# AdaptiveCity/deepdish

Measured on AMD Instinct MI355X. Metric: end-to-end frames/sec (detect+encode+track) at 640x480, higher is better.
Workload: dtype i8 (reference: uint8); encoder f16; 1 GPU; SSD-MobileNet-v1 uint8-quantised (300x300) + MARS-64x32x3 + deep_sort on synthetic 640x480 BGR frames, ~20 synthetic detections/frame (BASELINE.json configs[1]); streams_per_gpu=3072, worker_threads_per_gpu=2, parallelism=independent streams, 3072 per GPU in 2 worker groups, weights=seeded synthetic (seed 1234)

## Files before the change

deepdish_amd/csrc/mars_pair.hip:

```cpp
#include "mars_tail.h"

namespace {

typedef _Float16 h8 __attribute__((ext_vector_type(8)));
typedef float f4 __attribute__((ext_vector_type(4)));
typedef unsigned u4 __attribute__((ext_vector_type(4)));

__device__ __forceinline__ float elu(float v) {
    float e = __builtin_amdgcn_exp2f(v * 1.44269504088896340736f);
    e = __builtin_amdgcn_fmed3f(e, 0.f, 1.f);
    return __builtin_amdgcn_fmed3f(v, e - 1.f, 3.0e38f);
}

__device__ __forceinline__ void lds_fill16(const _Float16 *g, char *lds_wave_base) {
#if defined(__HIP_DEVICE_COMPILE__)
    __builtin_amdgcn_global_load_lds(g, lds_wave_base, 16, 0, 0);
#endif
}

__device__ __forceinline__ int frag_row(int a, int fr) { return (fr >> 2) * 8 + (a & 1) * 4 + (fr & 3); }

constexpr int PZ_B = 3072;
constexpr int PT64_B = 18 * 1024;
constexpr int PT32_B = 33 * 1024;
// ... 43 lines not shown
                    const size_t row = (size_t)(half * 32 + frag_row(a, fr)) * kpad;
                    wf[t][ks][a] = a32 ? *reinterpret_cast<const h8 *>(w + row + t * 32 + fq * 8)
                                       : *reinterpret_cast<const h8 *>(w + row + t * 64 + ks * 32 + fq * 8);
                }
#pragma unroll
        for (int a = 0; a < 2; ++a)
            wp[a] = FIRST ? *reinterpret_cast<const h8 *>(P.wp + (size_t)(half * 32 + frag_row(a, fr)) * P.kpad_p + fq * 8) : wf[0][0][a];
    }
#if defined(__HIP_DEVICE_COMPILE__)
#pragma unroll
    for (int t = 0; t < 9; ++t)
#pragma unroll
        for (int ks = 0; ks < 2; ++ks)
#pragma unroll
            for (int a = 0; a < 2; ++a) asm volatile("" ::"v"(wf[t][ks][a]));
    asm volatile("" ::"v"(wp[0]), "v"(wp[1]));
#endif

    const int n0 = blockIdx.x, nstep = gridDim.x;
    const int Kc = (P.n_img - n0 + nstep - 1) / nstep;

    const _Float16 *src[5];
    size_t stp[5];
    int n_dma;
    if constexpr (FIRST) {
        const int par = lane >> 5, pl = (lane >> 3) & 3, col = 2 * (lane & 7) + par;
#pragma unroll
        for (int h = 0; h < 4; ++h) {
            const int r = wave + 8 * h < 31 ? wave + 8 * h : 30;
            src[h] = col < 15 ? P.in + ((size_t)n0 * 31 + r) * 15 * P.cs_in + (size_t)col * P.cs_in + P.coff_in + pl * 8 : P.zero;
            stp[h] = col < 15 ? (size_t)nstep * 31 * 15 * P.cs_in : 0;
        }
        const int jr = lane >> 5, xx = lane & 7;
        src[4] = P.in2 + ((size_t)n0 * 31 + 2 * (2 * wave + jr)) * 15 * P.cs_in2 + (size_t)(2 * xx) * P.cs_in2 + P.coff_in2 + pl * 8;
        stp[4] = (size_t)nstep * 31 * 15 * P.cs_in2;
        n_dma = 5;
    } else {
        const int pl = lane >> 3, xx = lane & 7;
#pragma unroll
        for (int h = 0; h < 2; ++h) {
            src[h] = P.in + (((size_t)n0 * 16 + wave + 8 * h) * 8 + xx) * P.cs_in + P.coff_in + pl * 8;
            stp[h] = (size_t)nstep * 128 * P.cs_in;
            src[2 + h] = P.res + (((size_t)n0 * 16 + wave + 8 * h) * 8 + xx) * P.cs_res + P.coff_res + pl * 8;
            stp[2 + h] = (size_t)nstep * 128 * P.cs_res;
        }
        src[4] = P.zero; stp[4] = 0;
        n_dma = 4;
    }
    (void)n_dma;
    int dq = 0;
    auto issue = [&]() {
        char *T = smem + OFF_IN + (dq & 1) * TIN_B;
        if constexpr (FIRST) {
#pragma unroll
            for (int h = 0; h < 4; ++h) lds_fill16(src[h], T + ((wave + 8 * h < 31 ? wave + 8 * h : 30) + 1) * 1024);
            lds_fill16(src[4], smem + OFF_RAW + (dq & 1) * PRAW_B + wave * 1024);
        } else {
#pragma unroll
            for (int h = 0; h < 2; ++h) lds_fill16(src[h], T + (wave + 8 * h + 1) * 1024);
            const int rs = dq % 3;
#pragma unroll
            for (int h = 0; h < 2; ++h) lds_fill16(src[2 + h], smem + OFF_RES + rs * PPLAIN_B + (wave + 8 * h) * 1024);
        }
        ++dq;
        const bool more = dq < Kc;
#pragma unroll
        for (int h = 0; h < 5; ++h) src[h] += more ? stp[h] : 0;
    };
// ... 46 lines not shown
            } else {
                const unsigned tb = (unsigned)((stage == 0 ? OFF_IN + (cc & 1) * PT64_B : OFF_H + (cc & 1) * PT64_B) + 2 * F * 1024) + lo64;
                const unsigned bL = x == 0 ? ((tb - 16u) & 255u) : tb - 16u, bC = tb, bR = x == 7 ? ((tb + 16u) & 255u) : tb + 16u;
#if defined(__HIP_DEVICE_COMPILE__)
#define DD_RD(u_) do { constexpr int t_ = (u_) >> 1, ks_ = (u_) & 1, dy_ = t_ / 3, dx_ = t_ - dy_ * 3;                                             \
                       asm volatile("ds_read_b128 %0, %1 offset:%2" : "=&v"(X[(u_) & 3]) : "v"(dx_ == 0 ? bL : dx_ == 1 ? bC : bR), "n"(dy_ * 1024 + ks_ * 512) : "memory"); } while (0)
#define DD_UNIT(u_) do { if constexpr ((u_) + 3 < 18) DD_RD(((u_) + 3) % 18);                                                                      \
                         asm volatile("s_waitcnt lgkmcnt(%1)" : "+v"(X[(u_) & 3]) : "n"((u_) + 3 < 18 ? 3 : 17 - (u_)));                          \
                         _Pragma("unroll") for (int a = 0; a < 2; ++a) acc[a] = __builtin_amdgcn_mfma_f32_16x16x32_f16(wf[(u_) >> 1][(u_) & 1][a], X[(u_) & 3], acc[a], 0, 0, 0); } while (0)
                DD_RD(0); DD_RD(1); DD_RD(2);
                DD_UNIT(0); DD_UNIT(1); DD_UNIT(2); DD_UNIT(3); DD_UNIT(4); DD_UNIT(5); DD_UNIT(6); DD_UNIT(7); DD_UNIT(8);
                DD_UNIT(9); DD_UNIT(10); DD_UNIT(11); DD_UNIT(12); DD_UNIT(13); DD_UNIT(14); DD_UNIT(15); DD_UNIT(16); DD_UNIT(17);
#undef DD_UNIT
#undef DD_RD
#endif
            }
            float v[8];
#pragma unroll
            for (int i = 0; i < 4; ++i) { v[i] = acc[0][i] + ba0[i]; v[4 + i] = acc[1][i] + ba1[i]; }
            if (stage == 0) {
                h8 o;
#pragma unroll
                for (int i = 0; i < 8; ++i) o[i] = (_Float16)elu(v[i]);
                *reinterpret_cast<h8 *>(smem + OFF_H + (cc & 1) * PT64_B + ((2 * F + j + 1) * 64 + (half * 4 + fq) * 8 + x) * 16) = o;
            } else {
                const int rs = FIRST ? (cc & 1) : cc % 3;
                const h8 rv = *reinterpret_cast<const h8 *>(smem + OFF_RES + rs * PPLAIN_B + ((2 * F + j) * 64 + (half * 4 + fq) * 8 + x) * 16);
#pragma unroll
                for (int i = 0; i < 8; ++i) v[i] += (float)rv[i];
                const size_t m = (n * 16 + 2 * F + j) * 8 + x;
                h8 o;
#pragma unroll
                for (int i = 0; i < 8; ++i) o[i] = (_Float16)v[i];
                *reinterpret_cast<h8 *>(P.out + m * P.cs_out + P.coff_out + co) = o;
                const f4 s0 = *reinterpret_cast<const f4 *>(cst + 128 + co), s1 = *reinterpret_cast<const f4 *>(cst + 128 + co + 4);
                const f4 t0 = *reinterpret_cast<const f4 *>(cst + 192 + co), t1 = *reinterpret_cast<const f4 *>(cst + 192 + co + 4);
                h8 o2;
#pragma unroll
                for (int i = 0; i < 4; ++i) { o2[i] = (_Float16)elu(s0[i] * v[i] + t0[i]); o2[4 + i] = (_Float16)elu(s1[i] * v[4 + i] + t1[i]); }
                *reinterpret_cast<h8 *>(P.out2 + m * P.cs_out2 + P.coff_out2 + co) = o2;
            }
        }
    }
#if defined(__HIP_DEVICE_COMPILE__)
    asm volatile("s_waitcnt vmcnt(0)" ::: "memory");
#endif
}

template <bool FIRST>
int launch_pair(hipStream_t s, int device, const MarsPairP &P) {
    constexpr int lds = pair_lds_bytes(FIRST);
    static_assert(lds <= 160 * 1024, "LDS budget");
    static DevOnce once;
    const int rc = once.run(device, [&]() -> int {
        DD_HIP(hipFuncSetAttribute(reinterpret_cast<const void *>(&mars_pair64_k<FIRST>), hipFuncAttributeMaxDynamicSharedMemorySize, lds));
        return DD_OK;
    });
    if (rc != DD_OK) return rc;
    const int n_cu = dd_cu_count(device);
    const int grid = P.n_img < n_cu ? P.n_img : n_cu;
    hipLaunchKernelGGL((mars_pair64_k<FIRST>), dim3(grid), dim3(512), lds, s, P);
    DD_LAUNCH_CHECK();
    return DD_OK;
}

}

// ... 6 lines not shown
```

deepdish_amd/csrc/mars_tail.h:

```cpp
#pragma once
#include "common.h"

struct MarsWsP {
    const _Float16 *in;  int cs_in, coff_in;
    const _Float16 *in2; int cs_in2, coff_in2;
    const _Float16 *w;   int kpad;
    const _Float16 *w2;  int kpad2;
    const float *bias, *bias2;
    const _Float16 *res; int cs_res, coff_res;
    _Float16 *out;  int cs_out, coff_out;
    _Float16 *out2; int cs_out2, coff_out2;
    const float *aff2; int cout_pad;
    const _Float16 *zero;
    int n_img;
};

enum { MARS_WS_S1 = 0, MARS_WS_S1_RES = 1, MARS_WS_S2_PROJ = 2 };

int mars_ws128_launch(hipStream_t s, int device, const MarsWsP &P, int mode, int act, bool out2);

struct MarsPairP {
    const _Float16 *in;  int cs_in, coff_in;
    const _Float16 *in2; int cs_in2, coff_in2;
    const _Float16 *wa;  int kpad_a; const float *bias_a;
    const _Float16 *wp;  int kpad_p; const float *bias_p;
    const _Float16 *wb;  int kpad_b; const float *bias_b;
    const _Float16 *res; int cs_res, coff_res;
    _Float16 *out;  int cs_out, coff_out;
    _Float16 *out2; int cs_out2, coff_out2;
    const float *aff2; int cout_pad;
    const _Float16 *zero;
    int n_img;
};
int mars_pair64_launch(hipStream_t s, int device, const MarsPairP &P, bool first);
```

deepdish_amd/csrc/mars_tail.hip:

```cpp
#include "mars_tail.h"
#include <vector>

namespace {

typedef _Float16 h8 __attribute__((ext_vector_type(8)));
typedef float f4 __attribute__((ext_vector_type(4)));
typedef unsigned u4 __attribute__((ext_vector_type(4)));

enum { ACT_NONE = 0, ACT_ELU = 2 };

__device__ __forceinline__ float elu(float v) {
    float e = __builtin_amdgcn_exp2f(v * 1.44269504088896340736f);
    e = __builtin_amdgcn_fmed3f(e, 0.f, 1.f);
    return __builtin_amdgcn_fmed3f(v, e - 1.f, 3.0e38f);
}

__device__ __forceinline__ void lds_fill16(const _Float16 *g, char *lds_wave_base) {
#if defined(__HIP_DEVICE_COMPILE__)
    __builtin_amdgcn_global_load_lds(g, lds_wave_base, 16, 0, 0);
#endif
}

__device__ __forceinline__ int frag_row(int a, int fr) { return (fr >> 2) * 8 + (a & 1) * 4 + (fr & 3); }

// ... 51 lines not shown
                wf[t][ks][a] = *reinterpret_cast<const h8 *>(P.w + (size_t)(cg * 32 + frag_row(a, fr)) * P.kpad + t * CIN + kh * (CIN / 2) + ks * 32 + fq * 8);
    h8 wp[2];
    if constexpr (S2) {
#pragma unroll
        for (int a = 0; a < 2; ++a) wp[a] = *reinterpret_cast<const h8 *>(P.w2 + (size_t)(cg * 32 + frag_row(a, fr)) * P.kpad2 + kh * 32 + fq * 8);
    }

#if defined(__HIP_DEVICE_COMPILE__)
#pragma unroll
    for (int t = 0; t < 9; ++t)
#pragma unroll
        for (int ks = 0; ks < KS; ++ks)
#pragma unroll
            for (int a = 0; a < 2; ++a) asm volatile("" ::"v"(wf[t][ks][a]));
    if constexpr (S2) asm volatile("" ::"v"(wp[0]), "v"(wp[1]));
#endif

    const int n0 = blockIdx.x, nstep = gridDim.x;
    const int Kc = (P.n_img - n0 + nstep - 1) / nstep;

    int dq = 0, dq_slot = 0, dq_rslot = 0;
    const _Float16 *src_a, *src_b, *src_c;
    size_t step_a, step_b, step_c;
    if constexpr (!S2) {
        src_a = P.in + (size_t)n0 * 32 * P.cs_in + ((wave * 4 + (lane & 3)) * P.cs_in + P.coff_in + (lane >> 2) * 8);
        src_b = RES ? P.res + (size_t)n0 * 32 * P.cs_res + ((wave * 4 + (lane & 3)) * P.cs_res + P.coff_res + (lane >> 2) * 8) : P.zero;
        src_c = P.zero;
        step_a = (size_t)nstep * 32 * P.cs_in; step_b = (size_t)nstep * 32 * P.cs_res; step_c = 0;
    } else {
        const int par = lane >> 5, pl = (lane >> 2) & 7, col = 2 * (lane & 3) + par;
        src_a = P.in + (size_t)n0 * 128 * P.cs_in + ((wave * 8 + col) * P.cs_in + P.coff_in + pl * 8);
        src_b = src_a + (size_t)64 * P.cs_in;
        const int ch = (wave & 3) * 64 + lane;
        src_c = P.in2 + (size_t)n0 * 128 * P.cs_in2 + ((2 * ((ch >> 2) & 7) * 8 + 2 * (ch & 3)) * P.cs_in2 + P.coff_in2 + (ch >> 5) * 8);
        step_a = step_b = (size_t)nstep * 128 * P.cs_in; step_c = (size_t)nstep * 128 * P.cs_in2;
    }
    auto issue = [&]() {
        char *T = smem + OFF_T + dq_slot * TILE_B;
        if constexpr (!S2) {
            lds_fill16(src_a, T + (wave + 1) * 72 * 16);
            if constexpr (RES) lds_fill16(src_b, smem + OFF_A + dq_rslot * WS_RES_BYTES + wave * 72 * 16);
        } else {
            lds_fill16(src_a, T + wave * 68 * 16);
            lds_fill16(src_b, T + (wave + 8) * 68 * 16);
            lds_fill16(src_c, smem + OFF_A + dq_slot * WS_PRJ_BYTES + (wave & 3) * 1024);
        }
        ++dq;
        const bool more = dq < Kc;
        src_a += more ? step_a : 0;
        if constexpr (RES || S2) src_b += more ? step_b : 0;
        if constexpr (S2) src_c += more ? step_c : 0;
        dq_slot = dq_slot + 1 == NB ? 0 : dq_slot + 1;
        dq_rslot = dq_rslot + 1 == NBR ? 0 : dq_rslot + 1;
    };

    const unsigned lo = S2 ? (unsigned)((2 * yy * 68 + (kh * 4 + fq) * 4 + x) * 16) : (unsigned)((yy * 72 + (kh * 8 + fq) * 4 + x) * 16);
    const unsigned lo_prj = (unsigned)(((kh * 4 + fq) * 32 + yy * 4 + x) * 16);
    const unsigned lo_res = (unsigned)(((4 * kh + yy) * 72 + (cg * 4 + fq) * 4 + x) * 16);
    const int co = cg * 32 + fq * 8;
    const f4 b0 = *reinterpret_cast<const f4 *>(cst + co), b1 = *reinterpret_cast<const f4 *>(cst + co + 4);

    f4 keep[S2 ? 4 : 2];
    int slot = 0, rslot_prev = 0, rslot = 0;

    auto epilogue = [&](int cprev) {
        const char *Xp = smem + OFF_X + ((cprev & 1) * 8 + (wave ^ 4)) * XW_B + lane * 16;
        const size_t n = (size_t)(n0 + cprev * nstep);
        const size_t m = (n * 8 + 4 * kh + yy) * 4 + x;
// ... 209 lines not shown
```

deepdish_amd/csrc/net_priv.h:

```cpp
#pragma once
#include <map>
#include <utility>
#include <vector>
#include "common.h"

struct TensorDesc { int buf, h, w, c, cs, coff, dtype, pad; };

struct dd_net {
    dd_ctx *ctx = nullptr;
    int max_batch = 0;
    std::vector<int32_t> prog;
    std::vector<TensorDesc> tensors;
    std::vector<int64_t> buf_elems;
    std::vector<void *> bufs;
    std::vector<int> buf_dtype;
    int n_ops = 0, ops_off = 0;
    void *arena = nullptr;
    int64_t arena_bytes = 0;
    char *d_weights = nullptr;
    int64_t weight_bytes = 0;
    int in_h = 0, in_w = 0, out_tensor = -1;
    bool profile = false;
    int last_batch = 0;
    DevBuf slab;
    bool ssd_dec = false, yolo_dec = false;
    int dec_anchors = 0; float dec_thr = 0.f;
    float *d_anchors = nullptr, *dec_boxes = nullptr, *dec_score = nullptr, *dec_keys = nullptr; int *dec_cls = nullptr;
    bool slab_moved = false;
    _Float16 *d_zero = nullptr;
    std::vector<hipEvent_t> events;
    std::vector<int32_t> op_launch;
    std::vector<int32_t> op_variant;
    struct GraphEntry { int calls = 0; hipGraph_t graph = nullptr; hipGraphExec_t exec = nullptr; };
    bool use_graph = false;
    std::map<std::pair<const void *, int>, GraphEntry> graphs;
};

constexpr int OP_WORDS = 48;
constexpr int TENSOR_WORDS = 8;

enum { OP_INPUT = 1, OP_CONV = 2, OP_DWCONV = 3, OP_MAXPOOL = 4, OP_UPSAMPLE = 5, OP_FC = 6, OP_L2NORM = 7, OP_STEM = 8, OP_DWPW = 9 };
enum { OP_QCONV0 = 16, OP_QCONV = 17, OP_QDW = 18, OP_QDWPW = 19, OP_QSSD_DECODE = 20, OP_QADD = 21 };
enum { ACT_NONE = 0, ACT_RELU6 = 1, ACT_ELU = 2, ACT_SILU = 3, ACT_RELU = 4, ACT_SIGMOID = 5 };
enum { EPI_F16 = 0, EPI_F32 = 1, EPI_SSD_HEAD = 2, EPI_YOLO = 3 };
enum { DT_F16 = 0, DT_F32 = 1, DT_U8 = 2 };
enum { HINT_NONE = 0,
       HINT_NEXT_ONLY = 1,
       HINT_HOLD_UNIT = 2,
       HINT_NEXT_IS_PROJ = 3,
       HINT_PAIR_MEMBER = 4 };

enum OpWord {
    W_KIND = 0,
    W_SRC = 1,
    W_DST = 2,
    W_RES = 3,
    W_DST2 = 4,
    W_KH = 5,
    W_KW = 6,
    W_STRIDE = 7,
    W_PAD_T = 8,
    W_PAD_L = 9,
    W_CIN = 10,
    W_COUT = 11,
    W_COUT_PAD = 12,
// ... 123 lines not shown
```

deepdish_amd/csrc/nets.hip:

```cpp
#include <algorithm>
#include <cmath>
#include <cstdlib>
#include <map>
#include <string>
#include "common.h"
#include "ssd_dev.h"
#include "net_priv.h"
#include "mars_tail.h"

namespace {

typedef _Float16 h8 __attribute__((ext_vector_type(8)));
typedef _Float16 h4 __attribute__((ext_vector_type(4)));
typedef float f4 __attribute__((ext_vector_type(4)));

enum { OPK_DEFAULT = 0, OPK_FOLDED = 1, OPK_POOL_ROWS = 2, OPK_POOL_ROWS_STEM = 3, OPK_RES_UNIT = 4, OPK_SSD_FRONT = 5, OPK_C64_ROWS = 6, OPK_S2_ROWS = 7, OPK_CONV_WS = 8, OPK_WS_DW = 9, OPK_DWPW_ROWS = 10, OPK_SSD_HEAD_DEC = 11, OPK_RES_PAIR = 12, OPK_YOLO_HEAD_DEC = 13, OPK_MARS_WS = 14, OPK_FOLDED_PREV = 15, OPK_MARS_PAIR = 16, OPK_C64_STRIPS = 18, OPK_Q_FRONT = 19, OPK_Q_MID = 20, OPK_STEM_WIDE = 23 };

__device__ __forceinline__ float fast_sigmoid(float v) { return __builtin_amdgcn_rcpf(1.f + __expf(-v)); }

__device__ __forceinline__ float yolo_box_col(int o, float s, float px, float py, float stride, float aw, float ah, float img_w, float img_h) {
#pragma clang fp contract(off)
    if (o == 0) return (s * 2.f - 0.5f + px) * stride / img_w;
    if (o == 1) return (s * 2.f - 0.5f + py) * stride / img_h;
    if (o == 2) return (s * 2.f) * (s * 2.f) * aw / img_w;
// ... 6 lines not shown
        case ACT_ELU: {
            float e = __builtin_amdgcn_exp2f(v * 1.44269504088896340736f);
            e = __builtin_amdgcn_fmed3f(e, 0.f, 1.f);
            return __builtin_amdgcn_fmed3f(v, e - 1.f, 3.0e38f);
        }
        case ACT_SILU: {
            float r = v * fast_sigmoid(v);
#if defined(__HIP_DEVICE_COMPILE__)
            asm("" : "+v"(r));
#endif
            return r;
        }
        case ACT_RELU: return fmaxf(v, 0.f);
        case ACT_SIGMOID: return 1.f / (1.f + __expf(-v));
        default: return v;
    }
}

__device__ __forceinline__ float pool_max(float a, float b) {
#if defined(__HIP_DEVICE_COMPILE__)
    return __builtin_elementwise_maximum(a, b);
#else
    return a > b ? a : b;
#endif
}

struct ConvP {
    const _Float16 *in; int H, W, cs_in, coff_in, cin;
    const _Float16 *w; const float *bias; int kpad;
    int kh, kw, stride, pad_t, pad_l;
    int ho, wo, cout, m;
    int act;
    void *out; int cs_out, coff_out, epi;
    const _Float16 *res; int cs_res, coff_res;
    _Float16 *out2; int cs_out2, coff_out2; const float *aff2; int cout_pad;
    int post_aff;
    int splitk; float *slab;
    const _Float16 *zero;
    int p[6]; float f[8];
    int th, tw, tiles_x, tiles_y;
    const uint8_t *src8; float in_mean, in_scale;
    const _Float16 *dw_w; const float *dw_bias; int dw_act; int total_quads;
    const float *anchors; float *dec_boxes, *dec_score, *dec_keys; int *dec_cls; float dec_thr;
};


__device__ __forceinline__ void conv_epilogue(const ConvP &P, int m, int co, float v[4], int hw) {
    const f4 bv = *reinterpret_cast<const f4 *>(P.bias + co);
#pragma unroll
    for (int r = 0; r < 4; ++r) v[r] += bv[r];
    if (P.epi == EPI_YOLO) {
        const int n = m / hw, p = m - n * hw;
        const int py = p / P.wo, px = p - py * P.wo;
#pragma unroll
        for (int r = 0; r < 4; ++r) {
            const int ch = co + r;
            if (ch >= P.cout) continue;
            const int no = P.p[0];
            const int an = ch / no, o = ch - an * no;
            const float s = fast_sigmoid(v[r]);
            float val = s;
            if (o < 4) val = yolo_box_col(o, s, (float)px, (float)py, P.f[6], P.f[2 * an], P.f[2 * an + 1], P.f[7], (float)P.p[4]);
            const size_t row = (size_t)n * P.p[1] + P.p[2] + (size_t)an * hw + p;
            static_cast<float *>(P.out)[row * no + o] = val;
        }
        return;
// ... 55 lines not shown
#if defined(__HIP_DEVICE_COMPILE__)
    if (HI) asm("v_fma_mix_f32 %0, %1, %2, %0 op_sel:[1,1,0] op_sel_hi:[1,1,0]" : "+v"(acc) : "v"(x), "v"(w));
    else asm("v_fma_mix_f32 %0, %1, %2, %0 op_sel:[0,0,0] op_sel_hi:[1,1,0]" : "+v"(acc) : "v"(x), "v"(w));
#endif
    return acc;
}
__device__ __forceinline__ void dw_tap(float (&acc)[8], const h8 &x, const h8 &w) {
    const u4v_t xv = __builtin_bit_cast(u4v_t, x), wv = __builtin_bit_cast(u4v_t, w);
#pragma unroll
    for (int i = 0; i < 8; ++i)
        acc[i] = (i & 1) ? fma_mix_f16<1>(xv[i >> 1], wv[i >> 1], acc[i]) : fma_mix_f16<0>(xv[i >> 1], wv[i >> 1], acc[i]);
}

struct Epi8 { f4 b0, b1, s0, s1, t0, t1; };

__device__ __forceinline__ Epi8 epi8_load(const ConvP &P, int co) {
    Epi8 E;
    E.b0 = *reinterpret_cast<const f4 *>(P.bias + co);
    E.b1 = *reinterpret_cast<const f4 *>(P.bias + co + 4);
    E.s0 = E.s1 = E.t0 = E.t1 = f4{0.f, 0.f, 0.f, 0.f};
    if (P.out2) {
        E.s0 = *reinterpret_cast<const f4 *>(P.aff2 + co);
        E.s1 = *reinterpret_cast<const f4 *>(P.aff2 + co + 4);
        E.t0 = *reinterpret_cast<const f4 *>(P.aff2 + P.cout_pad + co);
        E.t1 = *reinterpret_cast<const f4 *>(P.aff2 + P.cout_pad + co + 4);
    }
    return E;
}

#ifndef DD_EPI_NT
#define DD_EPI_NT true
#endif
template <int ACT = -1, bool BIAS = true, int EF = -1, bool NT = DD_EPI_NT, bool TAIL = true>
__device__ __forceinline__ void conv_epilogue_f16x8(const ConvP &P, const Epi8 &E, int m, int co, float v[8], const h8 *res_pre = nullptr) {
    const int act = ACT < 0 ? P.act : ACT;
    const bool has_res = EF < 0 ? P.res != nullptr : EF >= 1, has_out2 = EF < 0 ? P.out2 != nullptr : EF == 1;
#pragma unroll
    for (int r = 0; r < 4; ++r) {
        v[r] = apply_act(BIAS ? v[r] + E.b0[r] : v[r], act);
        v[4 + r] = apply_act(BIAS ? v[4 + r] + E.b1[r] : v[4 + r], act);
    }
    if (has_res) {
        const h8 rv = res_pre ? *res_pre : *reinterpret_cast<const h8 *>(P.res + (size_t)m * P.cs_res + P.coff_res + co);
#pragma unroll
        for (int r = 0; r < 8; ++r) v[r] += (float)rv[r];
    }
    const bool tail = TAIL && co + 8 > P.cout;
    h8 o;
#pragma unroll
    for (int r = 0; r < 8; ++r) o[r] = (_Float16)v[r];
    if (tail) {
#pragma unroll
        for (int r = 0; r < 8; ++r)
            if (co + r >= P.cout) o[r] = (_Float16)0.f;
    }
    h8 *dst = reinterpret_cast<h8 *>(static_cast<_Float16 *>(P.out) + (size_t)m * P.cs_out + P.coff_out + co);
    if constexpr (NT) __builtin_nontemporal_store(o, dst);
    else *dst = o;
    if (has_out2) {
        h8 o2;
#pragma unroll
        for (int r = 0; r < 8; ++r) {
            const float sc = r < 4 ? E.s0[r] : E.s1[r - 4], sh = r < 4 ? E.t0[r] : E.t1[r - 4];
            o2[r] = (_Float16)apply_act(sc * v[r] + sh, ACT_ELU);
        }
        if (tail) {
#pragma unroll
            for (int r = 0; r < 8; ++r)
                if (co + r >= P.cout) o2[r] = (_Float16)0.f;
        }
        *reinterpret_cast<h8 *>(P.out2 + (size_t)m * P.cs_out2 + P.coff_out2 + co) = o2;
    }
}

template <int ACT = -1>
__device__ __forceinline__ void conv_epilogue_f16x8(const ConvP &P, int m, int co, float v[8]) {
    const Epi8 E = epi8_load(P, co);
    conv_epilogue_f16x8<ACT>(P, E, m, co, v);
}

template <int ACT, int BM, int BN, int T>
__device__ __forceinline__ void conv_finish_rows(const ConvP &P, const float *ot, int m0, int n0) {
    constexpr int OROW = BN + 4, G = BN / 8;
    static_assert(T % G == 0, "a thread keeps its channel group over the row loop");
    const int g = threadIdx.x % G, co = n0 + g * 8;
    if (co >= P.cout_pad) return;
    const Epi8 E = epi8_load(P, co);
    for (int pl = threadIdx.x / G; pl < BM; pl += T / G) {
        const int m = m0 + pl;
        if (m >= P.m) break;
        const f4 lo = *reinterpret_cast<const f4 *>(ot + pl * OROW + g * 8);
// ... 1387 lines not shown
            __builtin_amdgcn_sched_barrier(0);
#endif
            if (i + 1 < 4) rd(i + 1, X[(i + 1) & 1]);
#if defined(__HIP_DEVICE_COMPILE__)
            __builtin_amdgcn_sched_barrier(0);
#endif
#pragma unroll
            for (int dx = 0; dx < 3; ++dx)
#pragma unroll
                for (int cr = 0; cr < 2; ++cr) {
                    const int dy = i - cr;
                    if (dy < 0 || dy > 2) continue;
#pragma unroll
                    for (int a = 0; a < 2; ++a)
                        acc[cr][a] = __builtin_amdgcn_mfma_f32_16x16x32_f16(w[dy * 3 + dx][a], x[dx], acc[cr][a], 0, 0, 0);
                }
#if defined(__HIP_DEVICE_COMPILE__)
            __builtin_amdgcn_sched_barrier(0);
#endif
        }
    };
    f4 accC[2][2];
    int grC = -1;
    auto b_store = [&]() {
#pragma unroll
        for (int cr = 0; cr < 2; ++cr) {
            const int s = 2 * grC - 1 + cr;
            const int kk = (s + 1) >> 5, y = ((s + 1) & 31) - 1;
            if (y < 0 || fr >= W) continue;
            float o[8];
#pragma unroll
            for (int q = 0; q < 4; ++q) { o[q] = accC[cr][0][q]; o[4 + q] = accC[cr][1][q]; }
            const h8 rv = *reinterpret_cast<const h8 *>(resr + ((s + 1) & (RU_PRE_SLOTS - 1)) * RU_SLOT + offC);
            conv_epilogue_f16x8<ACT_NONE, false, 1, true, false>(P2B, EB, ((n0 + kk * nstep) * H + y) * W + fr, fq * 8, o, &rv);
        }
    };
    for (int g = 0; g < Gall; ++g) {
        const int gr = role ? g - 2 : g;
        const bool active = role ? (gr >= 0 && gr < GA) : (K > 0 && gr <= GA);
        if (grC >= 0) { b_store(); grC = -1; }
        if (active) {
            if (role == 0) { fill_pre(2 * gr + 5); fill_pre(2 * gr + 6); }
            {
                f4 acc[2][2] = {{bA0, bA1}, {bA0, bA1}};
                conv2(inr, 2 * gr, RU_PRE_SLOTS - 1, wA, acc);
#pragma unroll
                for (int cr = 0; cr < 2; ++cr) {
                    const int s = 2 * gr + cr;
                    const bool live = ((s + 1) & 31) != 0 && fr < W;
                    h8 o;
#pragma unroll
                    for (int q = 0; q < 4; ++q) {
                        o[q] = (_Float16)apply_act(acc[cr][0][q], actA);
                        o[4 + q] = (_Float16)apply_act(acc[cr][1][q], actA);
                    }
                    u4v_t ou = __builtin_bit_cast(u4v_t, o);
                    ou &= live ? 0xFFFFFFFFu : 0u;
                    *reinterpret_cast<u4v_t *>(h1r + (s & (RU_H1_SLOTS - 1)) * RU_SLOT + offC) = ou;
                }
            }
            {
                f4 acc[2][2] = {{EB.b0, EB.b1}, {EB.b0, EB.b1}};
                conv2(h1r, 2 * gr - 2, RU_H1_SLOTS - 1, wB, acc);
                h8 rv[2];
#pragma unroll
                for (int cr = 0; cr < 2; ++cr) rv[cr] = *reinterpret_cast<const h8 *>(resr + ((2 * gr + cr) & (RU_PRE_SLOTS - 1)) * RU_SLOT + offC);
                if (role == 0) {
// ... 2337 lines not shown
    *n_ops_host = n->n_ops;
    return DD_OK;
}

int dd_net_op_variants(dd_net *n, int32_t *codes_host, int cap, int *n_ops_host) {
    DD_REQUIRE(n && codes_host && n_ops_host, DD_E_ARG, "dd_net_op_variants: NULL argument");
    DD_REQUIRE(cap >= n->n_ops, DD_E_ARG, "dd_net_op_variants: cap %d < %d ops", cap, n->n_ops);
    for (int i = 0; i < n->n_ops; ++i) codes_host[i] = i < (int)n->op_variant.size() ? n->op_variant[i] : 0;
    *n_ops_host = n->n_ops;
    return DD_OK;
}

int dd_net_read(dd_net *n, int tensor, int n_img, void *dst, int dst_on_device, void *stream) {
    DD_REQUIRE(n && dst && n_img >= 0 && n_img <= n->max_batch, DD_E_ARG, "dd_net_read: bad argument");
    DD_DEVICE(n->ctx);
    const int t = tensor < 0 ? n->out_tensor : tensor;
    DD_REQUIRE(t >= 0 && t < (int)n->tensors.size(), DD_E_ARG, "dd_net_read: tensor %d out of range", t);
    const TensorDesc &d = n->tensors[t];
    DD_REQUIRE(!n->arena || t == n->out_tensor, DD_E_STATE, "dd_net_read: tensor %d of an engine whose buffers share memory by lifetime "
               "(dd_net_create_shared): only the output tensor outlives the forward", t);
    DD_REQUIRE(d.coff == 0, DD_E_ARG, "dd_net_read: tensor %d is a channel slice", t);
    for (int i = 0; i < n->n_ops && i < (int)n->op_launch.size(); ++i) {
        const OpView o = op(n, i);
        DD_REQUIRE(!(o.dst() == t && n->op_launch[i] == OPK_SSD_HEAD_DEC), DD_E_STATE,
                   "dd_net_read: tensor %d (the SSD head matrix) was not written: the head layers decoded in their epilogue "
                   "(dd_net_ssd_decode); read dd_net_ssd_decoded instead", t);
        DD_REQUIRE(!(o.dst() == t && n->op_launch[i] == OPK_YOLO_HEAD_DEC), DD_E_STATE,
                   "dd_net_read: tensor %d (the Detect matrix) was not written: the head layers reduced their rows in their epilogue "
                   "(dd_net_yolo_decode); read dd_net_yolo_decoded instead", t);
        DD_REQUIRE(!((o.dst() == t || o.dst2() == t) && n->op_launch[i] == OPK_FOLDED), DD_E_STATE,
                   "dd_net_read: tensor %d was not written by the last forward (op %d ran inside the next op's launch at this batch "
                   "size and its output stayed on chip); run a smaller batch or a program compiled without the fusion flags", t, i);
    }
    hipStream_t s = dd_pick_stream(n->ctx, stream);
    const size_t bytes = d.pad ? (size_t)n_img * (d.h + 2) * (d.w + 2) * d.cs
                               : (size_t)n_img * d.h * d.w * d.cs * dtype_size(d.dtype);
    if (!bytes) return DD_OK;
    DD_HIP(hipMemcpyAsync(dst, n->bufs[d.buf], bytes, dst_on_device ? hipMemcpyDeviceToDevice : hipMemcpyDeviceToHost, s));
    if (!dst_on_device) DD_HIP(hipStreamSynchronize(s));
    return DD_OK;
}

static int net_run_ops(dd_net *net, const uint8_t *input, int nimg, hipStream_t s);

int dd_net_use_graph(dd_net *net, int enable) {
    DD_REQUIRE(net, DD_E_ARG, "dd_net_use_graph: NULL net");
    DD_DEVICE(net->ctx);
    net->use_graph = enable != 0;
    if (!net->use_graph) net_drop_graphs(net);
    return DD_OK;
}

int dd_net_ssd_decode(dd_net *net, const float *anchors_host, int n_anchors, float score_thr, int enable) {
    DD_REQUIRE(net, DD_E_ARG, "dd_net_ssd_decode: NULL net");
    DD_DEVICE(net->ctx);
    net_drop_graphs(net);
    if (!enable) { net->ssd_dec = false; return DD_OK; }
    DD_REQUIRE(anchors_host && n_anchors > 0, DD_E_ARG, "dd_net_ssd_decode: anchors missing");
    int heads = 0;
    for (int i = 0; i < net->n_ops; ++i) {
        const OpView o = op(net, i);
        if (o.kind() == OP_CONV && o.epi() == EPI_SSD_HEAD) {
            DD_REQUIRE(o.aff_off() && o.p(1) == n_anchors && 4 + o.p(0) <= 96, DD_E_ARG,
                       "dd_net_ssd_decode: head op %d has no per-anchor weight copy, or %d anchors / %d classes do not fit", i, o.p(1), o.p(0));
            ++heads;
        }
// ... 198 lines not shown
    DD_REQUIRE(!h.unit_on && !h.pair_on && !h.stem_on && !h.pw_on && !h.input_on, DD_E_STATE,
               "dd_net_forward: op %d is folded into a neighbouring launch while an earlier op's launch is still held back", i);
    return DD_OK;
}

ConvP conv_params(const dd_net *net, const OpView &o, int nimg) {
    ConvP P;
    memset(&P, 0, sizeof(P));
    if (o.src() >= 0) {
        bind_tensor(net, o.src(), P.in, P.cs_in, P.coff_in);
        P.H = net->tensors[o.src()].h; P.W = net->tensors[o.src()].w;
    }
    P.cin = o.cin();
    P.kh = o.kh(); P.kw = o.kw(); P.stride = o.stride(); P.pad_t = o.pad_t(); P.pad_l = o.pad_l();
    P.cout = o.cout(); P.cout_pad = o.cout_pad(); P.kpad = o.kpad(); P.act = o.act(); P.epi = o.epi();
    P.w = blob<_Float16>(net, o.w_off());
    P.bias = blob<float>(net, o.bias_off());
    P.ho = o.ho(); P.wo = o.wo(); P.m = nimg * P.ho * P.wo;
    bind_tensor(net, o.dst(), P.out, P.cs_out, P.coff_out);
    if (o.res() >= 0) bind_tensor(net, o.res(), P.res, P.cs_res, P.coff_res);
    if (o.dst2() >= 0) {
        bind_tensor(net, o.dst2(), P.out2, P.cs_out2, P.coff_out2);
        P.aff2 = blob<float>(net, o.aff_off());
    }
    if (o.dst2() < 0 && o.has_aff()) {
        P.aff2 = blob<float>(net, o.aff_off());
        P.post_aff = 1;
    }
    for (int q = 0; q < 6; ++q) P.p[q] = o.p(q);
    for (int q = 0; q < 8; ++q) P.f[q] = o.f(q);
    return P;
}

void take_stem(ConvP &P, const ConvP &stem) {
    P.src8 = stem.src8; P.in_mean = stem.in_mean; P.in_scale = stem.in_scale;
    P.dw_w = stem.w; P.dw_bias = stem.bias; P.dw_act = stem.act;
}

bool unit_first_layer(const Run &r, int i, const OpView &o, const ConvP &P) {
    return o.hint() != HINT_NONE && !o.pool() && i + 1 < r.net->n_ops && r.nimg >= 160 && !P.res && !P.out2;
}

int run_input(Run &r, int i, const OpView &o) {
    dd_net *net = r.net; Held &h = r.held; hipStream_t s = r.s;
    const int dst = o.dst();
    const TensorDesc *td = &net->tensors[dst];
    _Float16 *out; int cs, coff;
    bind_tensor(net, dst, out, cs, coff);
    const int m = r.nimg * td->h * td->w;
    if (o.s2d() && o.hint() != HINT_NONE && !o.swap_rb() && cs == 32 && !coff && i + 1 < net->n_ops) {
        static const bool off = dd_env_int("DD_FOCUS_UNFUSED", 0) != 0;
        if (!off && rw_shape_plain(op(net, i + 1), dst, ACT_SILU) && td->w % 32 == 0) {
            h.input_on = true; h.input_mean = o.f(0); h.input_scale = o.f(1); h.input_op = i;
            net->op_launch[i] = OPK_FOLDED;
            return DD_OK;
        }
    }
    if (o.s2d() && cs >= 16 && cs % 8 == 0) {
        const int cpp = cs / 8;
        DD_REQUIRE((long long)m * cpp < (1ll << 31), DD_E_CAPACITY, "dd_net_forward: %d x %d input chunks", m, cpp);
        hipLaunchKernelGGL(input_s2d_chunks_k, dim3(dd_ceil_div(m * cpp, 256)), dim3(256), 0, s, r.input, net->in_h, net->in_w, o.swap_rb(),
                           o.f(0), o.f(1), m * cpp, cpp, out + coff, cs);
    } else
    hipLaunchKernelGGL(input_k, dim3(dd_ceil_div(m, 256)), dim3(256), 0, s, r.input, net->in_h, net->in_w, o.swap_rb(),
                       o.f(0), o.f(1), o.s2d(), m, out + coff, cs);
    DD_LAUNCH_CHECK();
// ... 42 lines not shown
            h.stem_on = false;
            take_stem(P, h.stem);
        } else if ((rc = flush(r, HELD_STEM)) != DD_OK) return rc;
    }
    if (unit_first_layer(r, i, o, P)) {
        if (h.pair_on && P.in != static_cast<const _Float16 *>(h.pair_b.out2) && (rc = flush(r, HELD_PAIR)) != DD_OK) return rc;
        h.unit_a = P; h.unit_op = i; h.unit_on = true;
        net->op_launch[i] = OPK_FOLDED;
        return DD_OK;
    }
    if (o.pool() && pool_rows_fusable(P, nimg)) net->op_launch[i] = P.src8 ? OPK_POOL_ROWS_STEM : OPK_POOL_ROWS;
    return launch_conv3x3_rw(r.s, P, nimg, o.pool(), r.device());
}

int run_conv(Run &r, int i, const OpView &o) {
    dd_net *net = r.net; Held &h = r.held; const int nimg = r.nimg; hipStream_t s = r.s;
    int rc;
    if (h.proj_done) {
        if ((rc = refuse_fold_while_held(h, i)) != DD_OK) return rc;
        h.proj_done = false; net->op_launch[i] = OPK_FOLDED_PREV;
        return DD_OK;
    }
    if (h.pair64_left > 0) {
        if ((rc = refuse_fold_while_held(h, i)) != DD_OK) return rc;
        if (--h.pair64_left > 0) { net->op_launch[i] = OPK_FOLDED; return DD_OK; }
        if ((rc = mars_pair64_launch(s, r.device(), h.pair64, h.pair64_first)) != DD_OK) return rc;
        net->op_launch[i] = OPK_MARS_PAIR;
        return DD_OK;
    }
    if (o.hint() == HINT_NEXT_IS_PROJ || o.hint() == HINT_PAIR_MEMBER) {
        const int n_ops = mars_pair_match(net, i, nimg, h.pair64, h.pair64_first);
        if (n_ops) {
            if ((rc = refuse_fold_while_held(h, i)) != DD_OK) return rc;
            h.pair64_left = n_ops - 1; net->op_launch[i] = OPK_FOLDED;
            return DD_OK;
        }
    }
    ConvP P = conv_params(net, o, nimg);
    DD_REQUIRE(!o.pool() || (P.kh == 3 && P.stride == 1 && P.cin == 32 && P.cout_pad == 32), DD_E_ARG,
               "dd_net_forward: fused pooling is only built for the 3x3 32->32 kernel");
    if (h.unit_on) {
        if (res_unit_fusable(h.unit_a, P, nimg)) {
            h.unit_on = false;
            P.zero = net->d_zero;
            if (h.pair_on) {
                if (res_pair_fusable(h.pair_a, h.pair_b, h.unit_a, P, nimg)) {
                    h.pair_on = false;
                    if ((rc = launch_res_pair(s, h.pair_a, h.pair_b, h.unit_a, P, nimg, r.device())) != DD_OK) return rc;
                    net->op_launch[i] = OPK_RES_PAIR;
                    return DD_OK;
                }
                if ((rc = flush(r, HELD_PAIR)) != DD_OK) return rc;
            }
            if (o.hint() == HINT_HOLD_UNIT && i + 2 < net->n_ops) {
                h.pair_a = h.unit_a; h.pair_b = P; h.pair_on = true; h.pair_op = i;
                net->op_launch[i] = OPK_FOLDED;
                return DD_OK;
            }
            if ((rc = launch_res_unit(s, h.unit_a, P, nimg, r.device())) != DD_OK) return rc;
            net->op_launch[i] = OPK_RES_UNIT;
            return DD_OK;
        }
        if (h.pair_on && (rc = flush(r, HELD_PAIR)) != DD_OK) return rc;
        if ((rc = flush(r, HELD_UNIT)) != DD_OK) return rc;
    }
    if (h.pair_on) {
        const bool next_a = rw_shape(P) && unit_first_layer(r, i, o, P) && P.in == static_cast<const _Float16 *>(h.pair_b.out2);
        if (!next_a && (rc = flush(r, HELD_PAIR)) != DD_OK) return rc;
    }
    if (P.epi == EPI_YOLO && net->yolo_dec && o.aff_off() && !o.has_aff()) {
        DD_REQUIRE(P.p[1] == net->dec_anchors, DD_E_ARG, "dd_net_forward: head of %d rows, decode set up for %d", P.p[1], net->dec_anchors);
        P.w = blob<_Float16>(net, o.aff_off());
        P.bias = blob<float>(net, o.aux_off());
        P.zero = net->d_zero;
        P.dec_boxes = net->dec_boxes; P.dec_score = net->dec_score; P.dec_cls = net->dec_cls;
        if ((rc = launch_yolo_head_dec(s, P)) != DD_OK) return rc;
        net->op_launch[i] = OPK_YOLO_HEAD_DEC;
        return DD_OK;
    }
    if (P.epi == EPI_SSD_HEAD && net->ssd_dec && o.aff_off() && !o.has_aff()) {
        DD_REQUIRE(P.p[1] == net->dec_anchors, DD_E_ARG, "dd_net_forward: head of %d anchors, decode set up for %d", P.p[1], net->dec_anchors);
        P.w = blob<_Float16>(net, o.aff_off());
        P.bias = blob<float>(net, o.aux_off());
        P.zero = net->d_zero;
        P.anchors = net->d_anchors; P.dec_boxes = net->dec_boxes; P.dec_score = net->dec_score; P.dec_keys = net->dec_keys;
        P.dec_cls = net->dec_cls; P.dec_thr = net->dec_thr;
        if ((rc = launch_ssd_head_dec(s, P)) != DD_OK) return rc;
        net->op_launch[i] = OPK_SSD_HEAD_DEC;
        return DD_OK;
    }
    const bool bk32 = o.bk() == 32;
    P.zero = net->d_zero;
    if (rw_shape(P)) return run_conv3x3_rw(r, i, o, P);
    if (mars_ws_s1_eligible(P)) {
        const MarsWsP Q = mars_ws_params(P, nimg);
        net->op_launch[i] = OPK_MARS_WS;
        return mars_ws128_launch(s, r.device(), Q, P.res ? MARS_WS_S1_RES : MARS_WS_S1, P.act, P.out2 != nullptr);
    } else if (o.hint() == HINT_NEXT_IS_PROJ && i + 1 < net->n_ops && mars_ws_s2_eligible(P) && mars_proj_follows(net, i, P)) {
        const OpView q = op(net, i + 1);
        MarsWsP Q = mars_ws_params(P, nimg);
        bind_tensor(net, q.src(), Q.in2, Q.cs_in2, Q.coff_in2);
        Q.w2 = blob<_Float16>(net, q.w_off()); Q.kpad2 = q.kpad();
        Q.bias2 = blob<float>(net, q.bias_off());
        bind_tensor(net, q.dst(), Q.out2, Q.cs_out2, Q.coff_out2);
        net->op_launch[i] = OPK_MARS_WS;
        rc = mars_ws128_launch(s, r.device(), Q, MARS_WS_S2_PROJ, P.act, false);
        h.proj_done = true;
        return rc;
    } else if (s2_rows_eligible(P, nimg, net->max_batch)) {
        net->op_launch[i] = OPK_S2_ROWS;
        return launch_conv3x3_s2_rows(s, P, nimg, r.device());
    } else if (c64_rows_eligible(P, nimg, net->max_batch)) {
        net->op_launch[i] = OPK_C64_ROWS;
        return launch_conv3x3_c64_rows(s, P, nimg, r.device());
    } else if (c64_strips_eligible(P, nimg, net->max_batch)) {
        net->op_launch[i] = OPK_C64_STRIPS;
        return launch_conv3x3_c64_strips(s, P, nimg, r.device());
    } else if (ws_eligible(P) && o.hint() != HINT_NONE && i + 1 < net->n_ops && P.act == ACT_RELU6) {
        h.pw = P; h.pw_op = i; h.pw_on = true; net->op_launch[i] = OPK_FOLDED;
        return DD_OK;
    } else if (ws_eligible(P)) {
        net->op_launch[i] = OPK_CONV_WS;
        return launch_ws(r, P);
    }
    return launch_conv_tiled(r, i, P, bk32);
}

int run_stem(Run &r, int i, const OpView &o) {
    dd_net *net = r.net; Held &h = r.held; const int nimg = r.nimg;
    const int dst = o.dst();
    const TensorDesc *td = &net->tensors[dst];
    ConvP P = conv_params(net, o, nimg);
    P.src8 = r.input; P.H = net->in_h; P.W = net->in_w; P.in_mean = o.f(0); P.in_scale = o.f(1);
    P.zero = net->d_zero;
// ... 157 lines not shown
    dd_net *net = r.net; const int nimg = r.nimg; hipStream_t s = r.s;
    const bool front_on = dd_env_int("DD_Q_FRONT", 1) != 0;
    const int front_min = dd_env_int("DD_Q_FRONT_MIN", 24);
    r.mid_on = dd_env_int("DD_Q_MID", 1) != 0 && nimg >= front_min;
    *first_op = 0;
    const bool front_ops = net->n_ops > 3 && op(net, 0).kind() == OP_QCONV0 && op(net, 1).kind() == OP_QDWPW && op(net, 2).kind() == OP_QDWPW;
    if (front_on && nimg >= front_min && front_ops) {
        if (net->profile) for (int k = 0; k < 3; ++k) DD_HIP(hipEventRecord(net->events[k], s));
        int ran = 0;
        const int rc = netq_run_front(net, op(net, 0).w, op(net, 1).w, op(net, 2).w, r.input, nimg, s, &ran);
        if (rc != DD_OK) return rc;
        if (ran) { *first_op = 3; net->op_launch[0] = OPK_FOLDED; net->op_launch[1] = OPK_FOLDED; net->op_launch[2] = OPK_Q_FRONT; }
    }
    return DD_OK;
}

int run_q_mid(Run &r, int i, int *ran) {
    dd_net *net = r.net;
    if (net->profile) DD_HIP(hipEventRecord(net->events[i + 1], r.s));
    *ran = 0;
    const int rc = netq_run_mid(net, op(net, i).w, op(net, i + 1).w, r.nimg, r.s, ran);
    if (rc != DD_OK) return rc;
    if (*ran) { net->op_launch[i] = OPK_FOLDED; net->op_launch[i + 1] = OPK_Q_MID; }
    return DD_OK;
}

}

extern "C" {

static int net_run_ops(dd_net *net, const uint8_t *input, int nimg, hipStream_t s) {
    net->op_launch.assign((size_t)net->n_ops, OPK_DEFAULT);
    net->op_variant.assign((size_t)net->n_ops, 0);
    Run r{net, input, nimg, s};
    Held &h = r.held;
    int first_op = 0;
    int rc = run_q_front(r, &first_op);
    if (rc != DD_OK) return rc;
    for (int i = first_op; i < net->n_ops; ++i) {
        if (net->profile) DD_HIP(hipEventRecord(net->events[i], s));
        const OpView o = op(net, i);
        const int kind = o.kind();
        DD_REQUIRE(!h.input_on || (kind == OP_CONV && i == h.input_op + 1), DD_E_STATE, "dd_net_forward: input op %d was folded into an op that did not take it", h.input_op);
        if (r.mid_on && kind == OP_QDWPW && i + 1 < net->n_ops && op(net, i + 1).kind() == OP_QDWPW) {
            int ran = 0;
            if ((rc = run_q_mid(r, i, &ran)) != DD_OK) return rc;
            if (ran) { ++i; continue; }
        }
        DD_REQUIRE((!h.wide_conv || kind == OP_CONV) && (!h.wide_pool || kind == OP_MAXPOOL), DD_E_STATE, "dd_net_forward: op %d does not take the first layer folded into it", i);
        if ((rc = flush_unclaimed(r, o)) != DD_OK) return rc;
        switch (kind) {
            case OP_INPUT: rc = run_input(r, i, o); break;
            case OP_CONV: rc = run_conv(r, i, o); break;
            case OP_STEM: rc = run_stem(r, i, o); break;
            case OP_DWPW: rc = run_dwpw(r, i, o); break;
            case OP_DWCONV: rc = run_dwconv(r, i, o); break;
            case OP_MAXPOOL: rc = run_pool(r, i, o); break;
            case OP_UPSAMPLE: rc = run_upsample(r, o); break;
            case OP_L2NORM: rc = run_l2norm(r, o); break;
            default: {
                int handled = 0;
                rc = netq_run_op(net, i, o.w, input, nimg, s, &handled);
                if (rc != DD_OK) return rc;
                DD_REQUIRE(handled, DD_E_ARG, "dd_net_forward: unknown op kind %d at %d", kind, i);
            }
        }
// ... 12 lines not shown
```

Measured before the change: 150,500 frames/s.

## Write MARS skip tensors compactly with only pixels the strided projection reads

When a residual block's output is read only by the next block's stride-2 1x1 projection, the writer now stores just the even-row/even-column pixels in a dense compact layout. The projection readers in the pair and ws128 kernels then load from that compact buffer. This is meant to cut global write and read traffic for the skip tensors. In exchange, the full tensor is no longer materialised, so dd_net_read refuses those tensors. An env flag DD_MARS_COMPACT_SKIP (on by default) turns it off.

```diff
diff --git a/deepdish_amd/csrc/mars_pair.hip b/deepdish_amd/csrc/mars_pair.hip
--- a/deepdish_amd/csrc/mars_pair.hip
+++ b/deepdish_amd/csrc/mars_pair.hip
@@ -99,8 +99,9 @@
             stp[h] = col < 15 ? (size_t)nstep * 31 * 15 * P.cs_in : 0;
         }
         const int jr = lane >> 5, xx = lane & 7;
-        src[4] = P.in2 + ((size_t)n0 * 31 + 2 * (2 * wave + jr)) * 15 * P.cs_in2 + (size_t)(2 * xx) * P.cs_in2 + P.coff_in2 + pl * 8;
-        stp[4] = (size_t)nstep * 31 * 15 * P.cs_in2;
+        src[4] = P.in2_compact ? P.in2 + (size_t)n0 * MARS_SKIP32_HALVES + (size_t)(((2 * wave + jr) * 8 + xx) * 32 + pl * 8)
+                               : P.in2 + ((size_t)n0 * 31 + 2 * (2 * wave + jr)) * 15 * P.cs_in2 + (size_t)(2 * xx) * P.cs_in2 + P.coff_in2 + pl * 8;
+        stp[4] = P.in2_compact ? (size_t)nstep * MARS_SKIP32_HALVES : (size_t)nstep * 31 * 15 * P.cs_in2;
         n_dma = 5;
     } else {
         const int pl = lane >> 3, xx = lane & 7;
@@ -213,7 +214,10 @@
                 h8 o;
 #pragma unroll
                 for (int i = 0; i < 8; ++i) o[i] = (_Float16)v[i];
-                *reinterpret_cast<h8 *>(P.out + m * P.cs_out + P.coff_out + co) = o;
+                const bool cmp = !FIRST && P.out_compact;
+                _Float16 *po = cmp ? P.out + n * MARS_SKIP64_HALVES + (size_t)((((half * 4 + fq) * 8 + F) * 4 + (x >> 1)) * 8)
+                                   : P.out + m * P.cs_out + P.coff_out + co;
+                if (!cmp || (j == 0 && (x & 1) == 0)) *reinterpret_cast<h8 *>(po) = o;
                 const f4 s0 = *reinterpret_cast<const f4 *>(cst + 128 + co), s1 = *reinterpret_cast<const f4 *>(cst + 128 + co + 4);
                 const f4 t0 = *reinterpret_cast<const f4 *>(cst + 192 + co), t1 = *reinterpret_cast<const f4 *>(cst + 192 + co + 4);
                 h8 o2;
diff --git a/deepdish_amd/csrc/mars_tail.h b/deepdish_amd/csrc/mars_tail.h
--- a/deepdish_amd/csrc/mars_tail.h
+++ b/deepdish_amd/csrc/mars_tail.h
@@ -13,7 +13,10 @@
     const float *aff2; int cout_pad;
     const _Float16 *zero;
     int n_img;
+    int in2_compact;
 };
+
+constexpr int MARS_SKIP32_HALVES = 16 * 8 * 32, MARS_SKIP64_HALVES = 8 * 8 * 4 * 8;
 
 enum { MARS_WS_S1 = 0, MARS_WS_S1_RES = 1, MARS_WS_S2_PROJ = 2 };
 
@@ -31,5 +34,7 @@
     const float *aff2; int cout_pad;
     const _Float16 *zero;
     int n_img;
+    int in2_compact;
+    int out_compact;
 };
 int mars_pair64_launch(hipStream_t s, int device, const MarsPairP &P, bool first);
diff --git a/deepdish_amd/csrc/mars_tail.hip b/deepdish_amd/csrc/mars_tail.hip
--- a/deepdish_amd/csrc/mars_tail.hip
+++ b/deepdish_amd/csrc/mars_tail.hip
@@ -107,8 +107,9 @@
         src_a = P.in + (size_t)n0 * 128 * P.cs_in + ((wave * 8 + col) * P.cs_in + P.coff_in + pl * 8);
         src_b = src_a + (size_t)64 * P.cs_in;
         const int ch = (wave & 3) * 64 + lane;
-        src_c = P.in2 + (size_t)n0 * 128 * P.cs_in2 + ((2 * ((ch >> 2) & 7) * 8 + 2 * (ch & 3)) * P.cs_in2 + P.coff_in2 + (ch >> 5) * 8);
-        step_a = step_b = (size_t)nstep * 128 * P.cs_in; step_c = (size_t)nstep * 128 * P.cs_in2;
+        src_c = P.in2_compact ? P.in2 + (size_t)n0 * MARS_SKIP64_HALVES + (size_t)(ch * 8)
+                              : P.in2 + (size_t)n0 * 128 * P.cs_in2 + ((2 * ((ch >> 2) & 7) * 8 + 2 * (ch & 3)) * P.cs_in2 + P.coff_in2 + (ch >> 5) * 8);
+        step_a = step_b = (size_t)nstep * 128 * P.cs_in; step_c = P.in2_compact ? (size_t)nstep * MARS_SKIP64_HALVES : (size_t)nstep * 128 * P.cs_in2;
     }
     auto issue = [&]() {
         char *T = smem + OFF_T + dq_slot * TILE_B;
diff --git a/deepdish_amd/csrc/net_priv.h b/deepdish_amd/csrc/net_priv.h
--- a/deepdish_amd/csrc/net_priv.h
+++ b/deepdish_amd/csrc/net_priv.h
@@ -31,6 +31,7 @@
     std::vector<hipEvent_t> events;
     std::vector<int32_t> op_launch;
     std::vector<int32_t> op_variant;
+    std::vector<uint8_t> skip_compact;
     struct GraphEntry { int calls = 0; hipGraph_t graph = nullptr; hipGraphExec_t exec = nullptr; };
     bool use_graph = false;
     std::map<std::pair<const void *, int>, GraphEntry> graphs;
diff --git a/deepdish_amd/csrc/nets.hip b/deepdish_amd/csrc/nets.hip
--- a/deepdish_amd/csrc/nets.hip
+++ b/deepdish_amd/csrc/nets.hip
@@ -62,6 +62,7 @@
     int ho, wo, cout, m;
     int act;
     void *out; int cs_out, coff_out, epi;
+    int out_compact;
     const _Float16 *res; int cs_res, coff_res;
     _Float16 *out2; int cs_out2, coff_out2; const float *aff2; int cout_pad;
     int post_aff;
@@ -183,7 +184,8 @@
 #define DD_EPI_NT true
 #endif
 template <int ACT = -1, bool BIAS = true, int EF = -1, bool NT = DD_EPI_NT, bool TAIL = true>
-__device__ __forceinline__ void conv_epilogue_f16x8(const ConvP &P, const Epi8 &E, int m, int co, float v[8], const h8 *res_pre = nullptr) {
+__device__ __forceinline__ void conv_epilogue_f16x8(const ConvP &P, const Epi8 &E, int m, int co, float v[8], const h8 *res_pre = nullptr,
+                                                    int out_mode = 0, h8 *out_at = nullptr, bool out_on = true) {
     const int act = ACT < 0 ? P.act : ACT;
     const bool has_res = EF < 0 ? P.res != nullptr : EF >= 1, has_out2 = EF < 0 ? P.out2 != nullptr : EF == 1;
 #pragma unroll
@@ -205,9 +207,11 @@
         for (int r = 0; r < 8; ++r)
             if (co + r >= P.cout) o[r] = (_Float16)0.f;
     }
-    h8 *dst = reinterpret_cast<h8 *>(static_cast<_Float16 *>(P.out) + (size_t)m * P.cs_out + P.coff_out + co);
-    if constexpr (NT) __builtin_nontemporal_store(o, dst);
-    else *dst = o;
+    h8 *dst = out_mode == 1 ? out_at : reinterpret_cast<h8 *>(static_cast<_Float16 *>(P.out) + (size_t)m * P.cs_out + P.coff_out + co);
+    if (out_mode == 0 || (out_mode == 1 && out_on)) {
+        if constexpr (NT) __builtin_nontemporal_store(o, dst);
+        else *dst = o;
+    }
     if (has_out2) {
         h8 o2;
 #pragma unroll
@@ -1661,7 +1665,14 @@
 #pragma unroll
             for (int q = 0; q < 4; ++q) { o[q] = accC[cr][0][q]; o[4 + q] = accC[cr][1][q]; }
             const h8 rv = *reinterpret_cast<const h8 *>(resr + ((s + 1) & (RU_PRE_SLOTS - 1)) * RU_SLOT + offC);
-            conv_epilogue_f16x8<ACT_NONE, false, 1, true, false>(P2B, EB, ((n0 + kk * nstep) * H + y) * W + fr, fq * 8, o, &rv);
+            const int m = ((n0 + kk * nstep) * H + y) * W + fr;
+            if (!P2B.out_compact) conv_epilogue_f16x8<ACT_NONE, false, 1, true, false>(P2B, EB, m, fq * 8, o, &rv);
+            else if (y & 1) conv_epilogue_f16x8<ACT_NONE, false, 1, true, false>(P2B, EB, m, fq * 8, o, &rv, 2);
+            else {
+                h8 *out_at = reinterpret_cast<h8 *>(static_cast<_Float16 *>(P2B.out) + (size_t)(n0 + kk * nstep) * MARS_SKIP32_HALVES +
+                                                    (size_t)(((y >> 1) * 8 + (fr >> 1)) * 32 + fq * 8));
+                conv_epilogue_f16x8<ACT_NONE, false, 1, true, false>(P2B, EB, m, fq * 8, o, &rv, 1, out_at, (fr & 1) == 0);
+            }
         }
     };
     for (int g = 0; g < Gall; ++g) {
@@ -4065,6 +4076,9 @@
                    "dd_net_read: tensor %d was not written by the last forward (op %d ran inside the next op's launch at this batch "
                    "size and its output stayed on chip); run a smaller batch or a program compiled without the fusion flags", t, i);
     }
+    DD_REQUIRE(!(t < (int)n->skip_compact.size() && n->skip_compact[t]), DD_E_STATE,
+               "dd_net_read: tensor %d was not written in full by the last forward (a compact skip image: only the pixels the next block's "
+               "projection reads, at this batch size); run a smaller batch or set DD_MARS_COMPACT_SKIP=0", t);
     hipStream_t s = dd_pick_stream(n->ctx, stream);
     const size_t bytes = d.pad ? (size_t)n_img * (d.h + 2) * (d.w + 2) * d.cs
                                : (size_t)n_img * d.h * d.w * d.cs * dtype_size(d.dtype);
@@ -4329,6 +4343,50 @@
     return P;
 }
 
+bool skip_compact_on() {
+    static const bool on = dd_env_int("DD_MARS_COMPACT_SKIP", 1) != 0;
+    return on;
+}
+int skip_sole_reader(const dd_net *net, int t, int writer) {
+    const int nt = (int)net->tensors.size();
+    if (t < 0 || t >= nt || t == net->out_tensor) return -1;
+    const TensorDesc &d = net->tensors[t];
+    if (d.coff != 0 || d.cs != d.c || d.dtype != DT_F16 || d.pad) return -1;
+    int reader = -1;
+    for (int k = 0; k < net->n_ops; ++k) {
+        const OpView w = op(net, k);
+        for (int a : {w.src(), w.res()})
+            if (a >= 0 && a < nt && net->tensors[a].buf == d.buf) {
+                if (reader >= 0 && reader != k) return -1;
+                reader = k;
+            }
+        for (int a : {w.dst(), w.dst2()})
+            if (k != writer && a >= 0 && a < nt && net->tensors[a].buf == d.buf) return -1;
+    }
+    return reader > writer ? reader : -1;
+}
+bool skip32_compact(const dd_net *net, int i, int nimg) {
+    if (!skip_compact_on()) return false;
+    const int t = op(net, i).dst(), k = skip_sole_reader(net, t, i);
+    if (k < 1 || op(net, k).src() != t) return false;
+    MarsPairP Q; bool first = false;
+    return mars_pair_match(net, k - 1, nimg, Q, first) == 3 && first;
+}
+bool skip64_compact(const dd_net *net, int nb, int nimg) {
+    if (!skip_compact_on()) return false;
+    const int t = op(net, nb).dst(), k = skip_sole_reader(net, t, nb);
+    if (k < 1 || op(net, k).src() != t || net->tensors[t].c != 64) return false;
+    const OpView a = op(net, k - 1);
+    if (a.kind() != OP_CONV || a.hint() != HINT_NEXT_IS_PROJ || a.pool() || a.src() < 0) return false;
+    const ConvP P = conv_params(net, a, nimg);
+    return mars_ws_s2_eligible(P) && mars_proj_follows(net, k - 1, P);
+}
+bool reads_skip_compact(const dd_net *net, const OpView &o) {
+    for (int a : {o.src(), o.res()})
+        if (a >= 0 && a < (int)net->skip_compact.size() && net->skip_compact[a]) return true;
+    return false;
+}
+
 void take_stem(ConvP &P, const ConvP &stem) {
     P.src8 = stem.src8; P.in_mean = stem.in_mean; P.in_scale = stem.in_scale;
     P.dw_w = stem.w; P.dw_bias = stem.bias; P.dw_act = stem.act;
@@ -4437,10 +4495,13 @@
         const int n_ops = mars_pair_match(net, i, nimg, h.pair64, h.pair64_first);
         if (n_ops) {
             if ((rc = refuse_fold_while_held(h, i)) != DD_OK) return rc;
+            if (h.pair64_first) h.pair64.in2_compact = net->skip_compact[op(net, i + 1).src()];
+            else if (skip64_compact(net, i + 1, nimg)) { h.pair64.out_compact = 1; net->skip_compact[op(net, i + 1).dst()] = 1; }
             h.pair64_left = n_ops - 1; net->op_launch[i] = OPK_FOLDED;
             return DD_OK;
         }
     }
+    DD_REQUIRE(!reads_skip_compact(net, o), DD_E_STATE, "dd_net_forward: op %d reads a tensor that was written as a compact skip image", i);
     ConvP P = conv_params(net, o, nimg);
     DD_REQUIRE(!o.pool() || (P.kh == 3 && P.stride == 1 && P.cin == 32 && P.cout_pad == 32), DD_E_ARG,
                "dd_net_forward: fused pooling is only built for the 3x3 32->32 kernel");
@@ -4451,6 +4512,7 @@
             if (h.pair_on) {
                 if (res_pair_fusable(h.pair_a, h.pair_b, h.unit_a, P, nimg)) {
                     h.pair_on = false;
+                    if (skip32_compact(net, i, nimg)) { P.out_compact = 1; net->skip_compact[o.dst()] = 1; }
                     if ((rc = launch_res_pair(s, h.pair_a, h.pair_b, h.unit_a, P, nimg, r.device())) != DD_OK) return rc;
                     net->op_launch[i] = OPK_RES_PAIR;
                     return DD_OK;
@@ -4505,6 +4567,7 @@
         const OpView q = op(net, i + 1);
         MarsWsP Q = mars_ws_params(P, nimg);
         bind_tensor(net, q.src(), Q.in2, Q.cs_in2, Q.coff_in2);
+        Q.in2_compact = net->skip_compact[q.src()];
         Q.w2 = blob<_Float16>(net, q.w_off()); Q.kpad2 = q.kpad();
         Q.bias2 = blob<float>(net, q.bias_off());
         bind_tensor(net, q.dst(), Q.out2, Q.cs_out2, Q.coff_out2);
@@ -4728,6 +4791,7 @@
 static int net_run_ops(dd_net *net, const uint8_t *input, int nimg, hipStream_t s) {
     net->op_launch.assign((size_t)net->n_ops, OPK_DEFAULT);
     net->op_variant.assign((size_t)net->n_ops, 0);
+    net->skip_compact.assign(net->tensors.size(), 0);
     Run r{net, input, nimg, s};
     Held &h = r.held;
     int first_op = 0;
```

After: 149,200 frames/s. Within noise of the previous version (-0.9%).
